# ami-iit/paper_gorbani_2025_humanoids_multi-rate-mpc-ironcub

Measured on AMD Instinct MI355X. Metric: MPC solves/sec (whole node) + p50 single-solve latency, iRonCub paper horizon, higher is better.
Workload: dtype f64

## Files before the change

paper_gorbani_2025_humanoids_multi-rate-mpc-ironcub_amd/build.py:

```python
from __future__ import annotations

import os
import shutil
import subprocess

HERE = os.path.dirname(os.path.abspath(__file__))
CSRC = os.path.join(HERE, "csrc")
LIB_PATH = os.path.join(HERE, "libvsmpc.so")
SOLVE = "vsmpc_kernels.hip"
SOURCES = [SOLVE, "vsmpc_dispatch.hip", "vsmpc_rollout.hip", "vsmpc_capi.hip", "vsmpc_capi_solve.hip", "vsmpc_capi_debug.hip",
           "vsmpc_capi_rollout.hip", "vsmpc_jet.hip", "vsmpc_provider.hip", "vsmpc_runtime.hip", "vsmpc_certify.hip"]
HEADERS = ["vsmpc_device.hpp", "vsmpc_launch.hpp", "vsmpc_host.hpp", "vsmpc_p0.hpp", "vsmpc_smem.hpp", "vsmpc_p1_syrk.hpp", "vsmpc_p1_struct.hpp",
           "vsmpc_p3.hpp", "vsmpc_p4.hpp", "vsmpc_p5.hpp", "vsmpc_panel_asm.inc",
           "vsmpc_structure.hpp", "vsmpc_rt_core.hpp", "vsmpc_rt_sens.hpp", "vsmpc_rt_adjoint.hpp", "vsmpc_solve_body.inc", "vsmpc_jet_device.hpp", "vsmpc_horizons.def", os.path.join("..", "..", "include", "vsmpc.h"),
           os.path.join("..", "..", "include", "vsmpc_jet.h")]


DEFAULT_HORIZONS = ((17, 7, 12), (34, 14, 24), (21, 9, 15))
HORIZONS_DEF = os.path.join(CSRC, "vsmpc_horizons.def")


def horizons():
    env = os.environ.get("VSMPC_HORIZONS", "").strip()
    if not env:
        return DEFAULT_HORIZONS
    out = []
    for item in env.split(";"):
        n, ns, hc = (int(v) for v in item.split(","))
        out.append((n, ns, hc))
    return tuple(out)


def write_horizons_def() -> bool:
    text = ("// Horizons (nIter, nIterSmall, controlHorizon) with a kernel instantiation: one X(...) line each.\n"
            "// Written by build.py (DEFAULT_HORIZONS or VSMPC_HORIZONS); the first two are BASELINE.json's configurations.\n"
            + "".join(f"X({n}, {ns}, {hc})\n" for n, ns, hc in horizons()))
    old = open(HORIZONS_DEF).read() if os.path.exists(HORIZONS_DEF) else None
    if old != text:
        with open(HORIZONS_DEF, "w") as f:
            f.write(text)
        return True
    return False


def _hipcc() -> str:
    for cand in (shutil.which("hipcc"), "/opt/rocm/bin/hipcc"):
        if cand and os.path.exists(cand):
            return cand
    raise RuntimeError("hipcc not found: the vsmpc HIP library cannot be built")


OBJ_DIR = os.path.join(HERE, "build")


SCHED_MAX_ILP = ["-mllvm", "-amdgpu-sched-strategy=max-ilp"]
SMALL_SCHED = SCHED_MAX_ILP


def _units():
    units = []
    for n, ns, hc in horizons():
        sched = SCHED_MAX_ILP if n <= 24 else []
        for st in (0, 1):
            units.append((f"kernels_{n}_{ns}_{hc}_{'diag' if st else 'prod'}", SOLVE,
                          [f"-DVS_TU_HORIZON={n},{ns},{hc}", f"-DVS_TU_STAMPS={st}"] + sched))
        for form in (0, 1):
            units.append((f"kernels_{n}_{ns}_{hc}_tuned_{'struct' if form else 'syrk'}", SOLVE,
                          [f"-DVS_TU_HORIZON={n},{ns},{hc}", "-DVS_TU_STAMPS=2", f"-DVS_TU_FORM={form}"] + sched))
        units.append((f"kernels_{n}_{ns}_{hc}_small", SOLVE, [f"-DVS_TU_HORIZON={n},{ns},{hc}", "-DVS_TU_STAMPS=3"] + SMALL_SCHED))
    for src in SOURCES:
        if src != SOLVE:
            units.append((os.path.splitext(src)[0], src, []))
    return units


def _deps(src):
    return [os.path.join(CSRC, src)] + [os.path.join(CSRC, h) for h in HEADERS] + [os.path.abspath(__file__)]


def _extra_flags():
    return os.environ.get("VSMPC_HIPCC_FLAGS", "").split()


def needs_build() -> bool:
    if not os.path.exists(LIB_PATH):
        return True
    t = os.path.getmtime(LIB_PATH)
    deps = [os.path.join(CSRC, s) for s in SOURCES + HEADERS] + [os.path.abspath(__file__)]
    return any(os.path.getmtime(d) > t for d in deps)


def build_library(force: bool = False, verbose: bool = False, jobs: int | None = None) -> str:
    from concurrent.futures import ThreadPoolExecutor
    changed = write_horizons_def()
    if not force and not changed and not needs_build():
        return LIB_PATH
    os.makedirs(OBJ_DIR, exist_ok=True)
    hipcc = _hipcc()
    base = [hipcc, "--offload-arch=gfx950", "-O3", "-std=c++17", "-fPIC", "-c"] + _extra_flags()
    if verbose:
        base.insert(1, "-Rpass-analysis=kernel-resource-usage")
    todo, objs = [], []
    for name, src, flags in _units():
        obj = os.path.join(OBJ_DIR, name + ".o")
        stamp = obj + ".flags"
        cmd = base + flags + [os.path.join(CSRC, src), "-o", obj]
        objs.append(obj)
        flagtext = " ".join(cmd)
        fresh = (not force and os.path.exists(obj) and os.path.exists(stamp) and open(stamp).read() == flagtext
                 and all(os.path.getmtime(d) <= os.path.getmtime(obj) for d in _deps(src)))
        if not fresh:
            todo.append((cmd, stamp, flagtext))

    def run(item):
        cmd, stamp, flagtext = item
        res = subprocess.run(cmd, capture_output=True, text=True)
        if res.returncode == 0:
            with open(stamp, "w") as f:
                f.write(flagtext)
        return cmd, res

    jobs = jobs or int(os.environ.get("VSMPC_BUILD_JOBS", "0")) or min(8, os.cpu_count() or 1)
    with ThreadPoolExecutor(max_workers=jobs) as pool:
        results = list(pool.map(run, todo))
    for cmd, res in results:
        if res.returncode != 0:
            raise RuntimeError("hipcc failed: " + " ".join(cmd) + "\n" + res.stdout + res.stderr)
        if verbose:
            print(res.stderr)
    keep = {os.path.basename(o) for o in objs}
    for f in os.listdir(OBJ_DIR):
        if f.endswith(".o") and f not in keep:
            os.remove(os.path.join(OBJ_DIR, f))
    link = [hipcc, "--offload-arch=gfx950", "-shared", "-fPIC", "-Wl,-rpath,/opt/rocm/lib", "-o", LIB_PATH] + objs
    res = subprocess.run(link, capture_output=True, text=True)
    if res.returncode != 0:
        raise RuntimeError("link failed:\n" + res.stdout + res.stderr)
    return LIB_PATH


def build_bindings(force: bool = False) -> str | None:
    try:
        import pybind11
    except ImportError:
        return None
    import sysconfig
    src = os.path.join(CSRC, "bindings_mpc.cpp")
    out = os.path.join(HERE, "bindingsMPC" + (sysconfig.get_config_var("EXT_SUFFIX") or ".so"))
    deps = [src, os.path.join(HERE, "..", "include", "VariableSamplingMPC.hpp"), os.path.join(HERE, "..", "include", "vsmpc.h")]
    if not force and os.path.exists(out) and all(os.path.getmtime(d) <= os.path.getmtime(out) for d in deps):
        return out
    build_library()
    cmd = ["g++", "-O2", "-std=c++17", "-shared", "-fPIC", f"-I{pybind11.get_include()}",
           f"-I{sysconfig.get_paths()['include']}", src, "-o", out, f"-L{HERE}", "-lvsmpc",
           "-Wl,-rpath,$ORIGIN", "-Wl,-rpath,/opt/rocm/lib"]
    res = subprocess.run(cmd, capture_output=True, text=True)
    if res.returncode != 0:
        raise RuntimeError("bindingsMPC build failed:\n" + res.stdout + res.stderr)
    return out


if __name__ == "__main__":
    print(build_library(force=True, verbose=True))
```

paper_gorbani_2025_humanoids_multi-rate-mpc-ironcub_amd/csrc/vsmpc_kernels.hip:

```cpp
#include <atomic>

#include "vsmpc_launch.hpp"
#include "vsmpc_p0.hpp"
#include "vsmpc_p1_syrk.hpp"
#include "vsmpc_p1_struct.hpp"
#include "vsmpc_p3.hpp"
#include "vsmpc_p4.hpp"
#include "vsmpc_p5.hpp"

#if !defined(VS_TU_HORIZON) || !defined(VS_TU_STAMPS)
#error "one unit per horizon and kind: -DVS_TU_HORIZON=N,NS,HC -DVS_TU_STAMPS=0|1, =2 -DVS_TU_FORM=0|1, or =3 (build.py)"
#endif
#if VS_TU_STAMPS == 2 && !defined(VS_TU_FORM)
#error "a unit of the tuned kind holds one condensing form: -DVS_TU_FORM=0|1"
#endif

namespace vsmpc {

template <class D, int K0 = 0, int K1 = NJC>
VS_DEV void p0_joint_reduction(double* __restrict__ sm, int lane) {
    using S = Smem<D>;
    static_assert(VSMPC_IN_LANG == VSMPC_IN_LLIN + 24, "Lambda_lin and Lambda_ang are adjacent in the record");
    const double* sIn = sm + S::oIn;
    const double* sCfg = sm + S::oCfg;
    double* sBj = sm + S::oBj;
    double* sQR = sm + S::oQR;
    const int c = lane < 6 ? lane : 6;
    double a[8];
    if constexpr (K0 == 0) {
#pragma unroll
        for (int j = 0; j < 8; ++j) {
            const double isw = fast_rsqrt(sCfg[CFG_WJ + j]);
            const double lam = sIn[VSMPC_IN_LLIN + (c < 6 ? c : 0) * 8 + j];
            const double bq = sCfg[CFG_WREG] * sIn[VSMPC_IN_QERR + j];
            a[j] = (c < 6 ? lam : bq) * isw;
            if (lane == 0) sQR[S::QR_ISW + j] = isw;
        }
    } else {
#pragma unroll
        for (int j = 0; j < 8; ++j) a[j] = sQR[S::QR_A + 8 * c + j];
    }
#pragma unroll
    for (int k = K0; k < K1; ++k) {
        double s0 = a[k] * a[k], s1 = 0.0;
#pragma unroll
        for (int i = k + 1; i < 8; i += 2) {
            s1 = fma(a[i], a[i], s1);
            if (i + 1 < 8) s0 = fma(a[i + 1], a[i + 1], s0);
        }
        const double s = s0 + s1;
        const double sk = readlane_f64(s, k), xk = readlane_f64(a[k], k);
        const bool nz = sk > 1e-300;
        const double rs = fast_rsqrt(nz ? sk : 1.0);
        const double nrm = nz ? sk * rs : 0.0;
        const double alpha = xk >= 0.0 ? -nrm : nrm;
        const double beta = nz ? rs * fast_rcp(nrm + fabs(xk)) : 0.0;
        double v[8];
        v[k] = xk - alpha;
#pragma unroll
        for (int i = k + 1; i < 8; ++i) v[i] = readlane_f64(a[i], k);
        double w0 = v[k] * a[k], w1 = 0.0;
#pragma unroll
        for (int i = k + 1; i < 8; i += 2) {
            w1 = fma(v[i], a[i], w1);
            if (i + 1 < 8) w0 = fma(v[i + 1], a[i + 1], w0);
        }
        const double w = (w0 + w1) * beta;
        const bool behind = lane > k;
#pragma unroll
        for (int i = k; i < 8; ++i) a[i] = behind ? fma(-w, v[i], a[i]) : a[i];
        a[k] = lane == k ? alpha : a[k];
        if (lane == 0) {
#pragma unroll
            for (int i = 0; i < 8; ++i) sQR[S::QR_V + 8 * k + i] = i >= k ? v[i] : 0.0;
            sQR[S::QR_BETA + k] = beta;
        }
    }
    if constexpr (K1 < NJC) {
        if (lane < 7) {
#pragma unroll
            for (int j = 0; j < 8; ++j) sQR[S::QR_A + 8 * lane + j] = a[j];
        }
        return;
    }
    if (lane < 6) {
        const int row = lane < 3 ? 3 + lane : 6 + lane;
#pragma unroll
        for (int k = 0; k < NJC; ++k) sBj[row * NJ + k] = k <= lane ? a[k] : 0.0;
    } else if (lane == 6) {
#pragma unroll
        for (int k = 0; k < NJC; ++k) sQR[S::QR_GY + k] = a[k];
        sQR[S::QR_NS + 0] = -a[6];
        sQR[S::QR_NS + 1] = -a[7];
    }
}

template <class D, int K1 = NJC, int K0 = 0>
VS_DEV void joint_expand(const double* __restrict__ sQR, const double* __restrict__ y, double (&u)[8]) {
    using S = Smem<D>;
    if constexpr (K1 == NJC) {
#pragma unroll
        for (int i = 0; i < NJC; ++i) u[i] = y[i];
        u[6] = sQR[S::QR_NS + 0];
        u[7] = sQR[S::QR_NS + 1];
    }
#pragma unroll
    for (int k = K1 - 1; k >= K0; --k) {
        double t = 0.0;
#pragma unroll
        for (int i = k; i < 8; ++i) t = fma(sQR[S::QR_V + 8 * k + i], u[i], t);
        t *= sQR[S::QR_BETA + k];
#pragma unroll
        for (int i = k; i < 8; ++i) u[i] = fma(-t, sQR[S::QR_V + 8 * k + i], u[i]);
    }
    if constexpr (K0 == 0) {
#pragma unroll
        for (int i = 0; i < 8; ++i) u[i] *= sQR[S::QR_ISW + i];
    }
}

struct SolveArgs {
    DevCfg cfg;
    const double* in;
    int batch;
    int pad_;
    double* xout;
    double* fmout;
    int* status_out;
    int* iters_out;
    double* dbgM;
    double* dbgL;
    unsigned long long* stamps;
};
VS_DEV const SolveArgs* late_args() {
    const SolveArgs* ka = reinterpret_cast<const SolveArgs*>(
        (const void*)__builtin_amdgcn_kernarg_segment_ptr());
    asm volatile("" : "+s"(ka));
    return ka;
}

template <class D, bool STAMPS, int FORM = 0>
__global__ __launch_bounds__(D::BLOCK, D::WG_PER_CU) void solve_kernel(DevCfg cfg, const double* __restrict__ in, int batch,
                                                         double* xout_, double* fmout_, int* status_out_,
                                                         int* iters_out_, double* dbgM_, double* dbgL_,
                                                         unsigned long long* stamps_) {
    constexpr bool TUNED = false;
    constexpr bool SMALL = false;
    const double* const tun = nullptr;
#include "vsmpc_solve_body.inc"
}

template <class D, int FORM = 0>
__global__ __launch_bounds__(D::BLOCK, D::WG_PER_CU) void solve_kernel_tuned(DevCfg cfg, const double* __restrict__ in, int batch,
                                                         double* xout_, double* fmout_, int* status_out_,
                                                         int* iters_out_, double* dbgM_, double* dbgL_,
                                                         unsigned long long* stamps_, const double* __restrict__ tun) {
    constexpr bool STAMPS = false;
    constexpr bool TUNED = true;
    constexpr bool SMALL = false;
#include "vsmpc_solve_body.inc"
}

template <class D, bool STAMPS>
__global__ __launch_bounds__(D::BLOCK, D::WG_PER_CU) void solve_kernel_small(DevCfg cfg, const double* __restrict__ in, int batch,
                                                         double* xout_, double* fmout_, int* status_out_,
                                                         int* iters_out_, double* dbgM_, double* dbgL_,
                                                         unsigned long long* stamps_) {
    constexpr bool TUNED = false;
    constexpr bool SMALL = true;
    constexpr int FORM = 1;
    const double* const tun = nullptr;
#include "vsmpc_solve_body.inc"
}

template <class D, bool STAMPS, int FORM>
static hipError_t launch_solve_f(const DevCfg& cfg, const double* d_in, int batch, double* d_x, double* d_fm,
                                 int* d_status, int* d_iters, double* dbgM, double* dbgL,
                                 unsigned long long* stamps, hipStream_t stream) {
    static std::atomic<bool> attr_set[MAX_DEVICES];
    constexpr size_t lds = FORM == 1 ? Smem<D>::bytes_struct : Smem<D>::bytes;
    const hipError_t e = allow_dynamic_lds(reinterpret_cast<const void*>(&solve_kernel<D, STAMPS, FORM>), attr_set, lds);
    if (e != hipSuccess) return e;
    hipLaunchKernelGGL((solve_kernel<D, STAMPS, FORM>), dim3(batch), dim3(D::BLOCK), lds, stream,
                       cfg, d_in, batch, d_x, d_fm, d_status, d_iters, dbgM, dbgL, stamps);
    return hipGetLastError();
}

template <int N, int NS, int HC, bool STAMPS>
hipError_t launch_solve_dims(int form, const DevCfg& cfg, const double* d_in, int batch, double* d_x, double* d_fm,
                             int* d_status, int* d_iters, double* dbgM, double* dbgL, unsigned long long* stamps,
                             hipStream_t stream) {
    using D = Dims<N, NS, HC>;
    if constexpr (D::STRUCT_P1) {
        if (form != 2) {
            return launch_solve_f<D, STAMPS, 1>(cfg, d_in, batch, d_x, d_fm, d_status, d_iters, dbgM, dbgL, stamps, stream);
        }
    }
    return launch_solve_f<D, STAMPS, 0>(cfg, d_in, batch, d_x, d_fm, d_status, d_iters, dbgM, dbgL, stamps, stream);
}

template <int N, int NS, int HC>
hipError_t launch_solve_small_dims(const DevCfg& cfg, const double* d_in, int batch, double* d_x, double* d_fm, int* d_status,
                                   int* d_iters, unsigned long long* stamps, hipStream_t stream) {
    using D = Dims<N, NS, HC>;
    if constexpr (!has_small_kind<D>()) {
        return hipErrorInvalidValue;
    } else {
        static std::atomic<bool> attr_set[2][MAX_DEVICES];
        constexpr size_t lds = Smem<D, true>::bytes_struct;
        static_assert(lds <= 160 * 1024, "the small-batch kind takes the LDS of one CU");
        auto go = [&](auto stc) {
            constexpr bool ST = decltype(stc)::value;
            const hipError_t e = allow_dynamic_lds(reinterpret_cast<const void*>(&solve_kernel_small<D, ST>), attr_set[ST], lds);
            if (e != hipSuccess) return e;
            hipLaunchKernelGGL((solve_kernel_small<D, ST>), dim3(batch), dim3(D::BLOCK), lds, stream, cfg, d_in, batch, d_x, d_fm,
                               d_status, d_iters, static_cast<double*>(nullptr), static_cast<double*>(nullptr), stamps);
            return hipGetLastError();
        };
        return stamps != nullptr ? go(std::true_type{}) : go(std::false_type{});
    }
}

template <int N, int NS, int HC, int FORM>
hipError_t launch_solve_tuned_dims(const DevCfg& cfg, const double* d_in, const double* d_tun, int batch, double* d_x,
                                   double* d_fm, int* d_status, int* d_iters, hipStream_t stream) {
    using D = Dims<N, NS, HC>;
    if constexpr (FORM == 1 && !D::STRUCT_P1) {
        return hipErrorInvalidValue;
    } else {
        static std::atomic<bool> attr_set[MAX_DEVICES];
        constexpr size_t lds = FORM == 1 ? Smem<D>::bytes_struct : Smem<D>::bytes;
        static_assert(D::WG_PER_CU < 2 || lds <= 80 * 1024, "the tuned kind keeps two workgroups per CU");
        const hipError_t e = allow_dynamic_lds(reinterpret_cast<const void*>(&solve_kernel_tuned<D, FORM>), attr_set, lds);
        if (e != hipSuccess) return e;
        hipLaunchKernelGGL((solve_kernel_tuned<D, FORM>), dim3(batch), dim3(D::BLOCK), lds, stream, cfg, d_in, batch, d_x, d_fm,
                           d_status, d_iters, static_cast<double*>(nullptr), static_cast<double*>(nullptr),
                           static_cast<unsigned long long*>(nullptr), d_tun);
        return hipGetLastError();
    }
}

#define VS_INSTANTIATE_SOLVE(N, NS, HC, ST)                                                                              \
    template hipError_t launch_solve_dims<N, NS, HC, ST>(int, const DevCfg&, const double*, int, double*, double*, int*, \
                                                         int*, double*, double*, unsigned long long*, hipStream_t);
#define VS_INSTANTIATE_TUNED(N, NS, HC, F)                                                                                 \
    template hipError_t launch_solve_tuned_dims<N, NS, HC, F>(const DevCfg&, const double*, const double*, int, double*, \
                                                              double*, int*, int*, hipStream_t);
#define VS_TU_APPLY(M, ...) M(__VA_ARGS__)
#define VS_INSTANTIATE_SMALL(N, NS, HC)                                                                              \
    template hipError_t launch_solve_small_dims<N, NS, HC>(const DevCfg&, const double*, int, double*, double*, int*, int*, \
                                                           unsigned long long*, hipStream_t);
#if VS_TU_STAMPS == 3
VS_TU_APPLY(VS_INSTANTIATE_SMALL, VS_TU_HORIZON)
#elif VS_TU_STAMPS == 2
VS_TU_APPLY(VS_INSTANTIATE_TUNED, VS_TU_HORIZON, VS_TU_FORM)
#elif VS_TU_STAMPS
VS_TU_APPLY(VS_INSTANTIATE_SOLVE, VS_TU_HORIZON, true)
#else
VS_TU_APPLY(VS_INSTANTIATE_SOLVE, VS_TU_HORIZON, false)
#endif

}
```

paper_gorbani_2025_humanoids_multi-rate-mpc-ironcub_amd/csrc/vsmpc_solve_body.inc:

```
#define VS_STAMP(i)                                                                         \
    do {                                                                                    \
        if constexpr (STAMPS) {                                                             \
            unsigned long long* st_ = late_args()->stamps;                                  \
            if (tid == 0 && st_ != nullptr) st_[size_t(blockIdx.x) * 16 + (i)] = __builtin_amdgcn_s_memtime(); \
        }                                                                                   \
    } while (0)
    unsigned long long t_acc[6] = {0, 0, 0, 0, 0, 0};
    unsigned long long t_mark = 0, stamp_t1 = 0, rt0 = 0;
    if constexpr (STAMPS) rt0 = __builtin_amdgcn_s_memrealtime();
#define VS_TIC()                                                     \
    do {                                                             \
        if constexpr (STAMPS) t_mark = __builtin_amdgcn_s_memtime(); \
    } while (0)
#define VS_TOC(i)                                                          \
    do {                                                                   \
        if constexpr (STAMPS) {                                            \
            const unsigned long long t_now = __builtin_amdgcn_s_memtime(); \
            t_acc[i] += t_now - t_mark;                                    \
            t_mark = t_now;                                                \
        }                                                                  \
    } while (0)
    using S = Smem<D, SMALL>;
    static_assert(!SMALL || (FORM == 1 && !TUNED), "the small-batch kind is the structured form of the shared kind");
    constexpr bool FUSED_DISPATCH = FORM == 1;
// ... 368 lines not shown
                    }
                }
            }
            if (nnodes == 1)
                for (int i = ptid; i < 2 * D::YS; i += D::BLOCK) sYm[18 * D::YS + i] = 0.0;
        };
        auto syrk_fixed = [&](auto nks_c, auto nact_c) __attribute__((always_inline)) {
            constexpr int NKS = decltype(nks_c)::value, NACT = decltype(nact_c)::value;
            if constexpr (NACT > 0) {
                double ha[SYRK_DIST], hb[SYRK_DIST];
#pragma unroll
                for (int ks = 0; ks < SYRK_DIST; ++ks) {
                    ha[ks] = slot_a(NACT - 1)[ks * 4 * D::YS];
                    hb[ks] = slot_b(NACT - 1)[ks * 4 * D::YS];
                }
#pragma unroll
                for (int q = NACT - 1; q >= 0; --q) {
                    const int qn = q > 0 ? q - 1 : 0;
                    syrk_slot<D, NKS, true>(acc[q], slot_a(q), slot_b(q), ha, hb, slot_a(qn), slot_b(qn));
                }
            }
        };
        if constexpr (UNROLLED) {
            static_for<0, NPASS>([&](auto mc) __attribute__((always_inline)) {
                constexpr int m = decltype(mc)::value;
                constexpr int nnodes = (2 * m + 1 < D::N) ? 2 : 1;
                VS_TIC();
                rec_pass(m, nnodes, sY);
                VS_TOC(0);
                __syncthreads();
                VS_TOC(1);
                syrk_fixed(std::integral_constant<int, nnodes == 2 ? 9 : 5>{}, std::integral_constant<int, nact_max<D>(m)>{});
                VS_TOC(2);
                __syncthreads();
            });
        } else {
            static_for<0, PassGroups<D>::count()>([&](auto gc) __attribute__((always_inline)) {
                constexpr PassGroups<D> pg{};
                constexpr int g = decltype(gc)::value;
#pragma unroll 1
                for (int m = pg.start[g]; m < pg.end[g]; ++m) {
                    VS_TIC();
                    rec_pass(m, pg.nks[g] == 9 ? 2 : 1, sY);
                    VS_TOC(0);
                    __syncthreads();
                    VS_TOC(1);
                    syrk_fixed(std::integral_constant<int, pg.nks[g]>{}, std::integral_constant<int, pg.nact[g]>{});
                    VS_TOC(2);
                    __syncthreads();
                }
            });
        }
        VS_TIC();
    }
    if constexpr (!FUSED_DISPATCH) VS_STAMP(2);
    VS_REFRESH_IDS();
    if constexpr (D::WG_PER_CU == 1) pin_tiles_agpr<TPW>(acc);

    constexpr int PVT = D::PVT;
    const int crow = (lane >> 4) * 17 + (lane & 15);
    const int lrow = (lane & 15) * 17 + (lane >> 4);
    double* dbgM = STAMPS ? late_args()->dbgM : nullptr;
    double* dbgL = STAMPS ? late_args()->dbgL : nullptr;
    double* dbgLi = dbgL != nullptr ? dbgL + size_t(inst) * D::NP * D::NP : nullptr;
    if (STAMPS && !FUSED_DISPATCH && dbgM != nullptr) {
#pragma unroll
        for (int q = 0; q < TPW; ++q) {
            if (kTileTab<D, PIPE>.forms(q * D::NWAVES + wave, wave)) {
                const int ti_q = kTileTab<D, PIPE>.ti[q * D::NWAVES + wave], tj_q = kTileTab<D, PIPE>.tj[q * D::NWAVES + wave];
                d4 tmp = acc[q];
                if (ti_q == tj_q || ti_q >= PVT) {
#pragma unroll
                    for (int r = 0; r < 4; ++r)
                        tmp[r] += input_cost_term<D>(sCfg, smem + S::oQR + S::QR_GY, sVprev, 16 * ti_q + (lane >> 4) + 4 * r,
                                                     16 * tj_q + (lane & 15));
                }
#pragma unroll
                for (int r = 0; r < 4; ++r) {
                    const int gr = 16 * ti_q + (lane >> 4) + 4 * r, gc = 16 * tj_q + (lane & 15);
                    if (gc <= gr) dbgM[size_t(inst) * D::NP * D::NP + size_t(gr) * D::NP + gc] = tmp[r];
                }
            }
        }
    }
    if constexpr (!FUSED_DISPATCH) VS_STAMP(3);
    VS_REFRESH_IDS();
    if constexpr (!FUSED_DISPATCH)
    switch (wave) {
        case 0: cholesky_wave<D, TPW, 0, STAMPS, PIPE>(sCfg, acc, Lb, sInvD, smem + S::oQR + S::QR_GY, sVprev, sFlags, sXinv, sW, dbgLi, lane, crow, lrow, sZ); break;
        case 1: cholesky_wave<D, TPW, 1, STAMPS, PIPE>(sCfg, acc, Lb, sInvD, smem + S::oQR + S::QR_GY, sVprev, sFlags, sXinv, sW, dbgLi, lane, crow, lrow, sZ); break;
        case 2: cholesky_wave<D, TPW, 2, STAMPS, PIPE>(sCfg, acc, Lb, sInvD, smem + S::oQR + S::QR_GY, sVprev, sFlags, sXinv, sW, dbgLi, lane, crow, lrow, sZ); break;
        default: cholesky_wave<D, TPW, 3, STAMPS, PIPE>(sCfg, acc, Lb, sInvD, smem + S::oQR + S::QR_GY, sVprev, sFlags, sXinv, sW, dbgLi, lane, crow, lrow, sZ); break;
    }
    static_assert(D::NWAVES == 4, "wave-specialised phases are instantiated for four wavefronts");
    if (STAMPS && dbgLi != nullptr) {
        if constexpr (!FUSED_DISPATCH) {
#pragma unroll
            for (int q = 0; q < TPW; ++q) {
                const int ti_q = kTileTab<D, PIPE>.ti[q * D::NWAVES + wave], tj_q = kTileTab<D, PIPE>.tj[q * D::NWAVES + wave];
                if (kTileTab<D, PIPE>.holds(q * D::NWAVES + wave, wave) && tj_q < PVT && ti_q > tj_q) {
#pragma unroll
                    for (int r = 0; r < 4; ++r)
                        dbgLi[size_t(16 * ti_q + (lane >> 4) + 4 * r) * D::NP + 16 * tj_q + (lane & 15)] = acc[q][r];
                }
            }
        }
        for (int e = tid; e < (D::NP - 16 * PVT) * (D::NP - 16 * PVT); e += D::BLOCK) {
            const int gr = 16 * PVT + e / (D::NP - 16 * PVT), gc = 16 * PVT + e % (D::NP - 16 * PVT);
            if (gc <= gr) dbgLi[size_t(gr) * D::NP + gc] = Lb[lower_at<D>(gr, gc)];
        }
    }

    VS_STAMP(4);
    VS_REFRESH_IDS();
    if constexpr (D::WG_PER_CU == 1) pin_tiles_agpr<TPW>(acc);
    const bool hold = sIn[VSMPC_IN_HOLD] != 0.0;
    constexpr int PV = D::PVT;
    auto init_corner_rhs = [&]() {
        if (tid >= 16 * PV && tid < D::NP) sW[tid] = tid < D::NZ ? -Lb[lower_at<D>(D::NZ, tid)] : 0.0;
    };
    init_corner_rhs();
    if (tid < D::NP) sZ[tid] = (hold && tid >= D::NZ - 4 && tid < D::NZ) ? sVprev[tid - (D::NZ - 4)] : 0.0;
    __syncthreads();

    auto sweep_tile = [&](int p, bool prescribed) {
        if (wave == 0) {
            const int j = lane & 15;
            const int gj = 16 * p + j;
            const double* Tpp = Lb + tile_off<D>(p, p) + j;
            double colv[16];
#pragma unroll
            for (int k = 0; k < 16; ++k) {
                const double t = Tpp[k * 17];
                colv[k] = k >= j ? t : 0.0;
            }
            double w = sW[gj];
            const bool fix = (gj >= D::NZ) || (gj >= D::NU && (prescribed || (hold && gj >= D::NZ - 4)));
            const double inv_eff = fix ? 0.0 : sInvD[gj];
            const double zadd = (fix && gj < D::NZ) ? sZ[gj] : 0.0;
            double z = 0.0;
#pragma unroll
            for (int k = 15; k >= 0; --k) {
                const double zk = readlane_f64(fma(w, inv_eff, zadd), k);
                z = (j == k) ? zk : z;
                w = fma(-colv[k], zk, w);
            }
            if (lane < 16) sZ[gj] = z;
        }
        __syncthreads();
        if (p > PV) {
            if (tid >= 16 * PV && tid < 16 * p) {
                const double* T = Lb + tile_off<D>(p, tid >> 4) + (tid & 15);
                const double* zp = sZ + 16 * p;
                double a2 = 0.0;
#pragma unroll
                for (int k = 0; k < 16; ++k) a2 += T[k * 17] * zp[k];
                sW[tid] -= a2;
            }
            __syncthreads();
        }
    };

    constexpr bool DUALQP = S::DUALQP;
    if constexpr (DUALQP) {
        constexpr int PL = D::NT - 1, KL = D::NZ - 16 * PL;
        static_assert(KL == D::NV - 16 && KL >= 4, "pins live in the last tile row");
        const double* X6 = sXinv + PV * D::TS;
        const double* L76 = Lb + tile_off<D>(PL, PV);
        const double* L77 = Lb + tile_off<D>(PL, PL);
        if (wave == 0) {
            const int j = lane & 15;
            const int gj = 16 * PL + j;
            const double* Tpp = L77 + j;
            double colv[KL], l76[KL], x6[16];
#pragma unroll
            for (int k = 0; k < KL; ++k) {
                const double t = Tpp[k * 17];
                colv[k] = k >= j ? t : 0.0;
                l76[k] = L76[k * 17 + j];
            }
#pragma unroll
            for (int i = 0; i < 16; ++i) x6[i] = X6[i * 17 + j];
            double w = sW[gj];
            double w6 = sW[16 * PV + j];
            const bool fix = (j >= KL) || (hold && j >= KL - 4);
            const double inv_eff = fix ? 0.0 : sInvD[gj];
            const double zadd = (fix && j < KL) ? sZ[gj] : 0.0;
            double z = 0.0;
#pragma unroll
            for (int k = KL - 1; k >= 0; --k) {
                const double zk = readlane_f64(fma(w, inv_eff, zadd), k);
                z = (j == k) ? zk : z;
                w = fma(-colv[k], zk, w);
                w6 = fma(-l76[k], zk, w6);
            }
            double z6 = 0.0;
#pragma unroll
            for (int i = 0; i < 16; ++i) z6 = fma(x6[i], readlane_f64(w6, i), z6);
            if (lane < 16) { sZ[gj] = z; sZ[16 * PV + j] = z6; }
        } else {
            dual_setup_beside_sweep<D>(wave, lane);
        }
    } else if constexpr (S::DUAL3) {
        static_assert(D::NT - 1 == PV + 2, "three throttle tile rows");
        double x2[16];
        const double* L22d = Lb + tile_off_c<D>(PV + 2, PV + 2);
        const double* inv2 = sInvD + D::NU + 32;
        if (wave == 1) tile_inverse_rows<0, 8>(L22d, inv2, x2, lane);
        sweep_tile(PV + 2, false);
        auto sweep_tile_x = [&](int p, const double* Xp) {
            if (wave == 0) {
                const int j = lane & 15;
                double z0 = 0.0, z1 = 0.0;
#pragma unroll
                for (int k = 0; k < 16; k += 2) {
                    z0 = fma(Xp[k * 17 + j], sW[16 * p + k], z0);
                    z1 = fma(Xp[(k + 1) * 17 + j], sW[16 * p + k + 1], z1);
                }
                if (lane < 16) sZ[16 * p + j] = z0 + z1;
            }
            __syncthreads();
            if (p > PV) {
                if (tid >= 16 * PV && tid < 16 * p) {
                    const double* T = Lb + tile_off<D>(p, tid >> 4) + (tid & 15);
                    const double* zp = sZ + 16 * p;
                    double a2 = 0.0;
#pragma unroll
                    for (int k = 0; k < 16; ++k) a2 += T[k * 17] * zp[k];
                    sW[tid] -= a2;
                }
                __syncthreads();
            }
        };
        if (wave == 1) tile_inverse_rows<8, 13>(L22d, inv2, x2, lane);
        sweep_tile_x(PV + 1, smem + S::oDual3T0);
        if (wave == 1) {
            tile_inverse_rows<13, 16>(L22d, inv2, x2, lane);
            if (lane < 16) {
#pragma unroll
                for (int i = 0; i < 16; ++i) smem[S::oDual3T1 + i * 17 + lane] = x2[i];
            }
        }
        sweep_tile_x(PV, sXinv + PV * D::TS);
    } else {
#pragma unroll 1
        for (int p = D::NT - 1; p >= PV; --p) sweep_tile(p, false);
    }
    if (wave == 0) {
        const bool valid = lane < D::NV;
        const double v = sZ[D::NU + (valid ? lane : 0)];
        const bool fixed = hold && lane >= D::NV - 4;
        const double tolv = 1e-12 * (1.0 + fabs(v));
        const bool viol = valid && !fixed && (v < sCfg[CFG_VMIN] - tolv || v > sCfg[CFG_VMAX] + tolv);
        const unsigned long long vm = __ballot(viol);
        if (lane == 0) { sFlags[3] = __popcll(vm); sFlags[1] = VSMPC_STATUS_SOLVED; sFlags[2] = 1; }
        if constexpr (DUALQP) {
            if (lane == 0) sFlags[4] = int(unsigned(vm));
        }
    }
    __syncthreads();
    const bool need_qp = sFlags[3] != 0;
    VS_STAMP(5);
    VS_REFRESH_IDS();

#ifdef VS_DIAG_QP
    for (int i = 0; i < 4; ++i) t_acc[i] = 0;
#endif
    if (need_qp) {
#ifdef VS_DIAG_QP
        box_qp<D>(sFlags[3], hold, wave, STAMPS ? t_acc : nullptr);
#else
        box_qp<D>(sFlags[3], hold, wave);
#endif
        __syncthreads();
        VS_STAMP(6);
        VS_REFRESH_IDS();
        if constexpr (D::NU % 16 != 0) {
            init_corner_rhs();
            __syncthreads();
#pragma unroll 1
            for (int p = D::NT - 1; p >= PV; --p) sweep_tile(p, true);
        }
    } else {
        VS_STAMP(6);
    }
    switch (wave) {
        case 0:
            if constexpr (PIPE) p5_wave0_jets<D>(smem, lane);
            else backsub_wave<D, TPW, 0, PIPE>(acc, sW, sZ, sXinv, sU, lane);
            break;
        case 1: backsub_wave<D, TPW, 1, PIPE>(acc, sW, sZ, sXinv, sU, lane); break;
        case 2: backsub_wave<D, TPW, 2, PIPE>(acc, sW, sZ, sXinv, sU, lane); break;
        default: backsub_wave<D, TPW, 3, PIPE>(acc, sW, sZ, sXinv, sU, lane); break;
    }
    if (tid < D::NV) sV[tid] = sZ[D::NU + tid];
    __syncthreads();

    VS_STAMP(7);
    VS_REFRESH_IDS();
#ifdef VS_DIAG_P6
    for (int i = 0; i < 4; ++i) t_acc[i] = 0;
    VS_TIC();
#define VS_P6_TOC(i) VS_TOC(i)
#else
#define VS_P6_TOC(i) do { } while (0)
#endif
    const SolveArgs* ka = late_args();
    double* xout = ka->xout;
    double* fmout = ka->fmout;
    int* status_out = ka->status_out;
    int* iters_out = ka->iters_out;
    double u8[8] = {0.0, 0.0, 0.0, 0.0, 0.0, 0.0, 0.0, 0.0};
    constexpr int JX_SPLIT = PIPE ? 3 : NJC;
    if (PIPE && wave == 3 && lane < D::HC) joint_expand<D, NJC, JX_SPLIT>(smem + S::oQR, sZ + NJC * lane, u8);
    {
        constexpr int ROWS = PIPE ? 6 : NX;
        constexpr int NE = ROWS * D::N, RND = (NE + D::BLOCK - 1) / D::BLOCK;
#pragma unroll
        for (int rd = 0; rd < RND; ++rd) {
            const int e0 = tid + rd * D::BLOCK, ec = e0 < NE ? e0 : NE - 1;
            const int k = ec / ROWS, rr = ec - k * ROWS;
            const int r = PIPE ? (rr < 3 ? 3 + rr : 6 + rr) : rr;
            const int e = NX * k + r;
            const int jb = joint_block_of_stage<D>(k);
            const int tb = throttle_block_of_stage<D>(k);
            const int vq = tb == 0 ? D::NV - 4 : 4 * (tb - 1);
            double f = sC[r];
#pragma unroll
            for (int c = 0; c < NJC; ++c) f += sBj[r * NJ + c] * sZ[NJC * jb + c];
#pragma unroll
            for (int c = 0; c < NTH; ++c) f += sBt[r * NTH + c] * sV[vq + c];
            if (e0 < NE) sF[e] = f;
        }
    }
    __syncthreads();
    VS_P6_TOC(0);
    {
        constexpr int CHK = D::N > 20 ? 9 : 6, NCH = (D::N + CHK - 1) / CHK;
        double jT = 0.0, jTd = 0.0, jon = 0.0, ja = 0.0, jb = 0.0;
        double Sk[9], hh[3] = {0.0, 0.0, 0.0};
        double cm0 = 0.0, cm1 = 0.0, cm2 = 0.0, cce = 0.0, cx = 0.0, cee = 0.0;
        const int hr0m = (lane & 1) ? 9 : 3;
        const int cg = lane / 3, cr = lane - 3 * cg;
        const int cxr = (cg ? 6 : 0) + cr, chr0 = cg ? 9 : 3, cer = (cg ? 23 : 20) + cr;
        constexpr bool JETS_EARLY = PIPE;
        constexpr int JOFF = JETS_EARLY ? 0 : 1;
        if (!JETS_EARLY && wave == 0 && lane < NTH) {
            jon = sA[(12 + lane) * NX + 16 + lane]; ja = sA[(16 + lane) * NX + 12 + lane]; jb = sA[(16 + lane) * NX + 16 + lane];
            jT = sIn[VSMPC_IN_X0 + 12 + lane]; jTd = sIn[VSMPC_IN_X0 + 16 + lane];
            sX[12 + lane] = jT;
            sX[16 + lane] = jTd;
        }
        if (wave == 1 && lane < 2) {
#pragma unroll
            for (int r = 0; r < 3; ++r) {
                hh[r] = sIn[VSMPC_IN_X0 + hr0m + r];
                sX[hr0m + r] = hh[r];
#pragma unroll
                for (int c = 0; c < 3; ++c) Sk[3 * r + c] = sA[(hr0m + r) * NX + hr0m + c];
            }
        }
        if (wave == 2 && lane < 6) {
            cm0 = sA[cxr * NX + chr0]; cm1 = sA[cxr * NX + chr0 + 1]; cm2 = sA[cxr * NX + chr0 + 2];
            cce = sC[cer];
            cx = sIn[VSMPC_IN_X0 + cxr]; cee = sIn[VSMPC_IN_X0 + cer];
            sX[cxr] = cx;
            sX[cer] = cee;
        }
        static_assert(D::NUO <= D::NWAVES * D::NP, "joint increments fit the partial-sum array");
        if (wave == 3 && lane < D::HC) {
            if constexpr (PIPE) joint_expand<D, JX_SPLIT, 0>(smem + S::oQR, sZ + NJC * lane, u8);
            else joint_expand<D>(smem + S::oQR, sZ + NJC * lane, u8);
#pragma unroll
            for (int i = 0; i < 8; ++i) sU[NJ * lane + i] = u8[i];
        }
        if (wave == 3 && xout != nullptr) {
            double2* xo = reinterpret_cast<double2*>(xout + size_t(inst) * D::NVAR);
            for (int i = lane; i < D::NUO / 2; i += 64) xo[D::NXS / 2 + i] = make_double2(sU[2 * i], sU[2 * i + 1]);
            if (lane < D::NV / 2) {
                const int e = 2 * lane, b = e >> 2, c = e & 3;
                const int q = b == 0 ? D::NV - 4 + c : 4 * (b - 1) + c;
                xo[(D::NXS + D::NUO) / 2 + lane] = make_double2(sV[q], sV[q + 1]);
            }
        }

        static_for<0, NCH + 1 + JOFF>([&](auto scst) __attribute__((always_inline)) {
            constexpr int st = decltype(scst)::value;
            if constexpr (!JETS_EARLY && st < NCH) {
                if (wave == 0 && lane < NTH) {
                    constexpr int k0 = st * CHK;
                    double fa[CHK], fb[CHK], dtk[CHK];
#pragma unroll
                    for (int u = 0; u < CHK; ++u) {
                        const int k = (k0 + u < D::N) ? k0 + u : D::N - 1;
                        fa[u] = sF[NX * k + 12 + lane];
                        fb[u] = sF[NX * k + 16 + lane];
                        dtk[u] = sDt[k];
                    }
#pragma unroll
                    for (int u = 0; u < CHK; ++u) {
                        const double dT = fma(jon, jTd, fa[u]);
                        const double dTd = fma(ja, jT, fma(jb, jTd, fb[u]));
                        jT = fma(dtk[u], dT, jT);
                        jTd = fma(dtk[u], dTd, jTd);
                        if (k0 + u < D::N) {
                            sX[NX * (k0 + u + 1) + 12 + lane] = jT;
                            sX[NX * (k0 + u + 1) + 16 + lane] = jTd;
                        }
                    }
                }
            }
            if constexpr (PIPE && st == 1) {
                if (wave == 3 && fmout != nullptr && lane < VSMPC_FM_SIZE) {
                    double v;
                    if (lane < 8) v = sU[lane];
                    else if (lane < 12) v = sV[D::NV - 4 + (lane - 8)];
                    else if (lane < 16) v = Jet::throttle_of_v(sV[D::NV - 4 + (lane - 12)]);
                    else if (lane < 20) v = sX[NX + 12 + (lane - 16)];
                    else v = sX[NX + 16 + (lane - 20)];
                    fmout[size_t(inst) * VSMPC_FM_SIZE + lane] = v;
                }
            }
            if constexpr (st >= JOFF && st - JOFF < NCH) {
                if (wave == 1) {
                    constexpr int k0 = (st - JOFF) * CHK;
                    constexpr int kn = k0 + CHK < D::N ? CHK : D::N - k0;
                    if (lane < 6 * kn) {
                        const int k = k0 + lane / 6, rr = lane % 6, row = rr < 3 ? 3 + rr : 6 + rr;
                        double gk = sF[NX * k + row];
#pragma unroll
                        for (int c = 0; c < NTH; ++c) gk = fma(sA[row * NX + 12 + c], sX[NX * k + 12 + c], gk);
                        sF[NX * k + row] = gk;
                    }
                    if (lane < 2) {
                        double gk[CHK][3], dtk[CHK];
#pragma unroll
                        for (int u = 0; u < CHK; ++u) {
                            const int k = (k0 + u < D::N) ? k0 + u : D::N - 1;
#pragma unroll
                            for (int r = 0; r < 3; ++r) gk[u][r] = sF[NX * k + hr0m + r];
                            dtk[u] = sDt[k];
                        }
#pragma unroll
                        for (int u = 0; u < CHK; ++u) {
                            double dh[3];
#pragma unroll
                            for (int r = 0; r < 3; ++r)
                                dh[r] = fma(Sk[3 * r], hh[0], fma(Sk[3 * r + 1], hh[1], fma(Sk[3 * r + 2], hh[2], gk[u][r])));
#pragma unroll
                            for (int r = 0; r < 3; ++r) hh[r] = fma(dtk[u], dh[r], hh[r]);
                            if (k0 + u < D::N) {
#pragma unroll
                                for (int r = 0; r < 3; ++r) sX[NX * (k0 + u + 1) + hr0m + r] = hh[r];
                            }
                        }
                    }
                }
            }
            if constexpr (st >= JOFF + 1 && st - JOFF - 1 < NCH) {
                if (wave == 2 && lane < 6) {
                    constexpr int k0 = (st - JOFF - 1) * CHK;
                    double hk[CHK][3], dtk[CHK];
#pragma unroll
                    for (int u = 0; u < CHK; ++u) {
                        const int k = (k0 + u < D::N) ? k0 + u : D::N - 1;
#pragma unroll
                        for (int c = 0; c < 3; ++c) hk[u][c] = sX[NX * k + chr0 + c];
                        dtk[u] = sDt[k];
                    }
#pragma unroll
                    for (int u = 0; u < CHK; ++u) {
                        const double dx = fma(cm0, hk[u][0], fma(cm1, hk[u][1], cm2 * hk[u][2]));
                        cee = fma(dtk[u], cx + cce, cee);
                        cx = fma(dtk[u], dx, cx);
                        if (k0 + u < D::N) {
                            sX[NX * (k0 + u + 1) + cxr] = cx;
                            sX[NX * (k0 + u + 1) + cer] = cee;
                        }
                    }
                }
            }
            if constexpr (st + 1 < NCH + 1 + JOFF) __syncthreads();
            if constexpr (st == 0) VS_P6_TOC(1);
        });
    }
    __syncthreads();
    VS_P6_TOC(2);
    VS_STAMP(8);
    VS_REFRESH_IDS();

    if (xout != nullptr) {
        double2* xo = reinterpret_cast<double2*>(xout + size_t(inst) * D::NVAR);
        for (int i = tid; i < D::NXS / 2; i += D::BLOCK) xo[i] = make_double2(sX[2 * i], sX[2 * i + 1]);
    }
    if (!PIPE && fmout != nullptr && tid < VSMPC_FM_SIZE) {
        double v;
        if (tid < 8) v = sU[tid];
        else if (tid < 12) v = sV[D::NV - 4 + (tid - 8)];
        else if (tid < 16) v = Jet::throttle_of_v(sV[D::NV - 4 + (tid - 12)]);
        else if (tid < 20) v = sX[NX + 12 + (tid - 16)];
        else v = sX[NX + 16 + (tid - 20)];
        fmout[size_t(inst) * VSMPC_FM_SIZE + tid] = v;
    }
    if (tid == 0) {
        int st = sFlags[1];
        if (sFlags[0]) st = VSMPC_STATUS_NUMERICAL;
        status_out[inst] = st;
        if (iters_out != nullptr) iters_out[inst] = sFlags[2];
    }
    VS_P6_TOC(3);
    VS_STAMP(9);
    if constexpr (STAMPS) {
        unsigned long long* st_ = late_args()->stamps;
        if (tid == 0 && st_ != nullptr) {
#if defined(VS_DIAG_P3) && !defined(VS_DIAG_P6)
            for (int i = 0; i < 4; ++i) t_acc[i] = vs_diag_p3[i];
#endif
            t_acc[5] = __builtin_amdgcn_s_memrealtime() - rt0;
            t_acc[4] = rt0;
            for (int i = 0; i < 6; ++i) st_[size_t(blockIdx.x) * 16 + 10 + i] = t_acc[i];
        }
    }
#undef VS_STAMP
#undef VS_REFRESH_IDS
#undef VS_TIC
#undef VS_TOC
```

Baseline: 8.157 million.

## Restructure final rollout phase into single-wave streamed chains without per-chunk barriers

Replaces the multi-wave chunked pipeline of the state rollout (jets on wave 0, angular momentum on wave 1, CoM on wave 2, separated by a __syncthreads per chunk) with a design where wave 0 first integrates the jet states, then one barrier, then a fused chain (momentum plus CoM in six lanes) streams through the horizon with double-buffered register preloads. The jet coupling term is folded into the parallel forcing computation ahead of time. This removes many block-wide barriers and the wave-to-wave handoff latency, at the cost of serialising the jet and chain recurrences on a single wave and doing more redundant per-lane arithmetic.

```diff
diff --git a/paper_gorbani_2025_humanoids_multi-rate-mpc-ironcub_amd/build.py b/paper_gorbani_2025_humanoids_multi-rate-mpc-ironcub_amd/build.py
--- a/paper_gorbani_2025_humanoids_multi-rate-mpc-ironcub_amd/build.py
+++ b/paper_gorbani_2025_humanoids_multi-rate-mpc-ironcub_amd/build.py
@@ -11,7 +11,7 @@
 SOURCES = [SOLVE, "vsmpc_dispatch.hip", "vsmpc_rollout.hip", "vsmpc_capi.hip", "vsmpc_capi_solve.hip", "vsmpc_capi_debug.hip",
            "vsmpc_capi_rollout.hip", "vsmpc_jet.hip", "vsmpc_provider.hip", "vsmpc_runtime.hip", "vsmpc_certify.hip"]
 HEADERS = ["vsmpc_device.hpp", "vsmpc_launch.hpp", "vsmpc_host.hpp", "vsmpc_p0.hpp", "vsmpc_smem.hpp", "vsmpc_p1_syrk.hpp", "vsmpc_p1_struct.hpp",
-           "vsmpc_p3.hpp", "vsmpc_p4.hpp", "vsmpc_p5.hpp", "vsmpc_panel_asm.inc",
+           "vsmpc_p3.hpp", "vsmpc_p4.hpp", "vsmpc_p5.hpp", "vsmpc_p6.hpp", "vsmpc_panel_asm.inc",
            "vsmpc_structure.hpp", "vsmpc_rt_core.hpp", "vsmpc_rt_sens.hpp", "vsmpc_rt_adjoint.hpp", "vsmpc_solve_body.inc", "vsmpc_jet_device.hpp", "vsmpc_horizons.def", os.path.join("..", "..", "include", "vsmpc.h"),
            os.path.join("..", "..", "include", "vsmpc_jet.h")]
 
diff --git a/paper_gorbani_2025_humanoids_multi-rate-mpc-ironcub_amd/csrc/vsmpc_kernels.hip b/paper_gorbani_2025_humanoids_multi-rate-mpc-ironcub_amd/csrc/vsmpc_kernels.hip
--- a/paper_gorbani_2025_humanoids_multi-rate-mpc-ironcub_amd/csrc/vsmpc_kernels.hip
+++ b/paper_gorbani_2025_humanoids_multi-rate-mpc-ironcub_amd/csrc/vsmpc_kernels.hip
@@ -7,6 +7,7 @@
 #include "vsmpc_p3.hpp"
 #include "vsmpc_p4.hpp"
 #include "vsmpc_p5.hpp"
+#include "vsmpc_p6.hpp"
 
 #if !defined(VS_TU_HORIZON) || !defined(VS_TU_STAMPS)
 #error "one unit per horizon and kind: -DVS_TU_HORIZON=N,NS,HC -DVS_TU_STAMPS=0|1, =2 -DVS_TU_FORM=0|1, or =3 (build.py)"
diff --git a/paper_gorbani_2025_humanoids_multi-rate-mpc-ironcub_amd/csrc/vsmpc_p6.hpp b/paper_gorbani_2025_humanoids_multi-rate-mpc-ironcub_amd/csrc/vsmpc_p6.hpp
--- /dev/null
+++ b/paper_gorbani_2025_humanoids_multi-rate-mpc-ironcub_amd/csrc/vsmpc_p6.hpp
@@ -0,0 +1,122 @@
+#pragma once
+#include "vsmpc_p5.hpp"
+
+namespace vsmpc {
+
+template <class D>
+struct P6Groups {
+    static constexpr int GRP = D::N <= 18 ? D::N : 9;
+    static constexpr int NG = (D::N + GRP - 1) / GRP;
+};
+
+template <class D>
+VS_DEV void p6_jets_stream(const double* __restrict__ sIn, const double* __restrict__ sA, const double* __restrict__ sF,
+                           const double* __restrict__ sDt, double* __restrict__ sX, int lane) {
+    constexpr int GRP = P6Groups<D>::GRP, NG = P6Groups<D>::NG;
+    if (lane < NTH) {
+        const double jon = sA[(12 + lane) * NX + 16 + lane], ja = sA[(16 + lane) * NX + 12 + lane], jb = sA[(16 + lane) * NX + 16 + lane];
+        double jT = sIn[VSMPC_IN_X0 + 12 + lane], jTd = sIn[VSMPC_IN_X0 + 16 + lane];
+        sX[12 + lane] = jT;
+        sX[16 + lane] = jTd;
+        double fa[2][GRP], fb[2][GRP], dtk[2][GRP];
+        auto load = [&](auto gcst) __attribute__((always_inline)) {
+            constexpr int g = decltype(gcst)::value, b = g & 1;
+#pragma unroll
+            for (int u = 0; u < GRP; ++u) {
+                const int k = (g * GRP + u < D::N) ? g * GRP + u : D::N - 1;
+                fa[b][u] = sF[NX * k + 12 + lane];
+                fb[b][u] = sF[NX * k + 16 + lane];
+                dtk[b][u] = sDt[k];
+            }
+        };
+        load(std::integral_constant<int, 0>{});
+        static_for<0, NG>([&](auto gcst) __attribute__((always_inline)) {
+            constexpr int g = decltype(gcst)::value, b = g & 1;
+            if constexpr (g + 1 < NG) load(std::integral_constant<int, g + 1>{});
+#pragma unroll
+            for (int u = 0; u < GRP; ++u) {
+                if (g * GRP + u < D::N) {
+                    const double dT = fma(jon, jTd, fa[b][u]);
+                    const double dTd = fma(ja, jT, fma(jb, jTd, fb[b][u]));
+                    jT = fma(dtk[b][u], dT, jT);
+                    jTd = fma(dtk[b][u], dTd, jTd);
+                    sX[NX * (g * GRP + u + 1) + 12 + lane] = jT;
+                    sX[NX * (g * GRP + u + 1) + 16 + lane] = jTd;
+                }
+            }
+        });
+    }
+}
+
+struct P6Chain {
+    double Sk[9], hh[3];
+    double cm0, cm1, cm2, cce, cx, cee;
+    int hr0, xr, er, r;
+};
+
+template <class D>
+VS_DEV void p6_chain_init(P6Chain& ch, const double* __restrict__ sIn, const double* __restrict__ sA,
+                          const double* __restrict__ sC, double* __restrict__ sX, int lane) {
+    const int g = lane / 3;
+    ch.r = lane - 3 * g;
+    ch.hr0 = g ? 9 : 3;
+    ch.xr = (g ? 6 : 0) + ch.r;
+    ch.er = (g ? 23 : 20) + ch.r;
+#pragma unroll
+    for (int r = 0; r < 3; ++r) {
+        ch.hh[r] = sIn[VSMPC_IN_X0 + ch.hr0 + r];
+#pragma unroll
+        for (int c = 0; c < 3; ++c) ch.Sk[3 * r + c] = sA[(ch.hr0 + r) * NX + ch.hr0 + c];
+    }
+    ch.cm0 = sA[ch.xr * NX + ch.hr0]; ch.cm1 = sA[ch.xr * NX + ch.hr0 + 1]; ch.cm2 = sA[ch.xr * NX + ch.hr0 + 2];
+    ch.cce = sC[ch.er];
+    ch.cx = sIn[VSMPC_IN_X0 + ch.xr]; ch.cee = sIn[VSMPC_IN_X0 + ch.er];
+    sX[ch.hr0 + ch.r] = sIn[VSMPC_IN_X0 + ch.hr0 + ch.r];
+    sX[ch.xr] = ch.cx;
+    sX[ch.er] = ch.cee;
+}
+
+template <class D, class Mid>
+VS_DEV void p6_chain_stream(P6Chain& ch, const double* __restrict__ sF, const double* __restrict__ sDt,
+                            double* __restrict__ sX, Mid&& after_preload) {
+    constexpr int GRP = P6Groups<D>::GRP, NG = P6Groups<D>::NG;
+    double gk[2][GRP][3], dtk[2][GRP];
+    auto load = [&](auto gcst) __attribute__((always_inline)) {
+        constexpr int g = decltype(gcst)::value, b = g & 1;
+#pragma unroll
+        for (int u = 0; u < GRP; ++u) {
+            const int k = (g * GRP + u < D::N) ? g * GRP + u : D::N - 1;
+#pragma unroll
+            for (int r = 0; r < 3; ++r) gk[b][u][r] = sF[NX * k + ch.hr0 + r];
+            dtk[b][u] = sDt[k];
+        }
+    };
+    load(std::integral_constant<int, 0>{});
+    after_preload();
+    const bool r0 = ch.r == 0, r1 = ch.r == 1;
+    static_for<0, NG>([&](auto gcst) __attribute__((always_inline)) {
+        constexpr int g = decltype(gcst)::value, b = g & 1;
+        if constexpr (g + 1 < NG) load(std::integral_constant<int, g + 1>{});
+#pragma unroll
+        for (int u = 0; u < GRP; ++u) {
+            if (g * GRP + u < D::N) {
+                const double dt = dtk[b][u];
+                const double dx = fma(ch.cm0, ch.hh[0], fma(ch.cm1, ch.hh[1], ch.cm2 * ch.hh[2]));
+                ch.cee = fma(dt, ch.cx + ch.cce, ch.cee);
+                ch.cx = fma(dt, dx, ch.cx);
+                double dh[3];
+#pragma unroll
+                for (int r = 0; r < 3; ++r)
+                    dh[r] = fma(ch.Sk[3 * r], ch.hh[0], fma(ch.Sk[3 * r + 1], ch.hh[1], fma(ch.Sk[3 * r + 2], ch.hh[2], gk[b][u][r])));
+#pragma unroll
+                for (int r = 0; r < 3; ++r) ch.hh[r] = fma(dt, dh[r], ch.hh[r]);
+                double* xn = sX + NX * (g * GRP + u + 1);
+                xn[ch.hr0 + ch.r] = r0 ? ch.hh[0] : (r1 ? ch.hh[1] : ch.hh[2]);
+                xn[ch.xr] = ch.cx;
+                xn[ch.er] = ch.cee;
+            }
+        }
+    });
+}
+
+}
diff --git a/paper_gorbani_2025_humanoids_multi-rate-mpc-ironcub_amd/csrc/vsmpc_solve_body.inc b/paper_gorbani_2025_humanoids_multi-rate-mpc-ironcub_amd/csrc/vsmpc_solve_body.inc
--- a/paper_gorbani_2025_humanoids_multi-rate-mpc-ironcub_amd/csrc/vsmpc_solve_body.inc
+++ b/paper_gorbani_2025_humanoids_multi-rate-mpc-ironcub_amd/csrc/vsmpc_solve_body.inc
@@ -694,8 +694,15 @@
     for (int i = 0; i < 4; ++i) t_acc[i] = 0;
     VS_TIC();
 #define VS_P6_TOC(i) VS_TOC(i)
+#define VS_P6_PRELOAD_DONE()                      \
+    do {                                          \
+        __builtin_amdgcn_sched_barrier(0);        \
+        __builtin_amdgcn_s_waitcnt(0xc07f);       \
+        __builtin_amdgcn_sched_barrier(0);        \
+    } while (0)
 #else
 #define VS_P6_TOC(i) do { } while (0)
+#define VS_P6_PRELOAD_DONE() do { } while (0)
 #endif
     const SolveArgs* ka = late_args();
     double* xout = ka->xout;
@@ -705,59 +712,57 @@
     double u8[8] = {0.0, 0.0, 0.0, 0.0, 0.0, 0.0, 0.0, 0.0};
     constexpr int JX_SPLIT = PIPE ? 3 : NJC;
     if (PIPE && wave == 3 && lane < D::HC) joint_expand<D, NJC, JX_SPLIT>(smem + S::oQR, sZ + NJC * lane, u8);
+    auto input_term = [&](int r, int k) __attribute__((always_inline)) {
+        const int jb = joint_block_of_stage<D>(k);
+        const int tb = throttle_block_of_stage<D>(k);
+        const int vq = tb == 0 ? D::NV - 4 : 4 * (tb - 1);
+        double f = sC[r];
+#pragma unroll
+        for (int c = 0; c < NJC; ++c) f += sBj[r * NJ + c] * sZ[NJC * jb + c];
+#pragma unroll
+        for (int c = 0; c < NTH; ++c) f += sBt[r * NTH + c] * sV[vq + c];
+        return f;
+    };
+    if constexpr (!PIPE) {
+        if (wave == 0) {
+            constexpr int NEJ = 8 * D::N, RNDJ = (NEJ + 63) / 64;
+#pragma unroll
+            for (int rd = 0; rd < RNDJ; ++rd) {
+                const int e0 = lane + rd * 64, ec = e0 < NEJ ? e0 : NEJ - 1;
+                const int k = ec >> 3, r = 12 + (ec & 7);
+                const double f = input_term(r, k);
+                if (e0 < NEJ) sF[NX * k + r] = f;
+            }
+            p6_jets_stream<D>(sIn, sA, sF, sDt, sX, lane);
+        }
+        __syncthreads();
+    }
+    P6Chain ch;
+    if constexpr (PIPE) {
+        if (wave == 0 && lane < 6) p6_chain_init<D>(ch, sIn, sA, sC, sX, lane);
+    }
     {
-        constexpr int ROWS = PIPE ? 6 : NX;
-        constexpr int NE = ROWS * D::N, RND = (NE + D::BLOCK - 1) / D::BLOCK;
+        constexpr int NE = 6 * D::N, RND = (NE + D::BLOCK - 1) / D::BLOCK;
 #pragma unroll
         for (int rd = 0; rd < RND; ++rd) {
             const int e0 = tid + rd * D::BLOCK, ec = e0 < NE ? e0 : NE - 1;
-            const int k = ec / ROWS, rr = ec - k * ROWS;
-            const int r = PIPE ? (rr < 3 ? 3 + rr : 6 + rr) : rr;
-            const int e = NX * k + r;
-            const int jb = joint_block_of_stage<D>(k);
-            const int tb = throttle_block_of_stage<D>(k);
-            const int vq = tb == 0 ? D::NV - 4 : 4 * (tb - 1);
-            double f = sC[r];
-#pragma unroll
-            for (int c = 0; c < NJC; ++c) f += sBj[r * NJ + c] * sZ[NJC * jb + c];
-#pragma unroll
-            for (int c = 0; c < NTH; ++c) f += sBt[r * NTH + c] * sV[vq + c];
-            if (e0 < NE) sF[e] = f;
+            const int k = ec / 6, rr = ec - k * 6;
+            const int r = rr < 3 ? 3 + rr : 6 + rr;
+            double gk = input_term(r, k);
+#pragma unroll
+            for (int c = 0; c < NTH; ++c) gk = fma(sA[r * NX + 12 + c], sX[NX * k + 12 + c], gk);
+            if (e0 < NE) sF[NX * k + r] = gk;
         }
     }
     __syncthreads();
     VS_P6_TOC(0);
     {
-        constexpr int CHK = D::N > 20 ? 9 : 6, NCH = (D::N + CHK - 1) / CHK;
-        double jT = 0.0, jTd = 0.0, jon = 0.0, ja = 0.0, jb = 0.0;
-        double Sk[9], hh[3] = {0.0, 0.0, 0.0};
-        double cm0 = 0.0, cm1 = 0.0, cm2 = 0.0, cce = 0.0, cx = 0.0, cee = 0.0;
-        const int hr0m = (lane & 1) ? 9 : 3;
-        const int cg = lane / 3, cr = lane - 3 * cg;
-        const int cxr = (cg ? 6 : 0) + cr, chr0 = cg ? 9 : 3, cer = (cg ? 23 : 20) + cr;
-        constexpr bool JETS_EARLY = PIPE;
-        constexpr int JOFF = JETS_EARLY ? 0 : 1;
-        if (!JETS_EARLY && wave == 0 && lane < NTH) {
-            jon = sA[(12 + lane) * NX + 16 + lane]; ja = sA[(16 + lane) * NX + 12 + lane]; jb = sA[(16 + lane) * NX + 16 + lane];
-            jT = sIn[VSMPC_IN_X0 + 12 + lane]; jTd = sIn[VSMPC_IN_X0 + 16 + lane];
-            sX[12 + lane] = jT;
-            sX[16 + lane] = jTd;
-        }
-        if (wave == 1 && lane < 2) {
-#pragma unroll
-            for (int r = 0; r < 3; ++r) {
-                hh[r] = sIn[VSMPC_IN_X0 + hr0m + r];
-                sX[hr0m + r] = hh[r];
-#pragma unroll
-                for (int c = 0; c < 3; ++c) Sk[3 * r + c] = sA[(hr0m + r) * NX + hr0m + c];
-            }
-        }
-        if (wave == 2 && lane < 6) {
-            cm0 = sA[cxr * NX + chr0]; cm1 = sA[cxr * NX + chr0 + 1]; cm2 = sA[cxr * NX + chr0 + 2];
-            cce = sC[cer];
-            cx = sIn[VSMPC_IN_X0 + cxr]; cee = sIn[VSMPC_IN_X0 + cer];
-            sX[cxr] = cx;
-            sX[cer] = cee;
+        if (wave == 0 && lane < 6) {
+            if constexpr (!PIPE) p6_chain_init<D>(ch, sIn, sA, sC, sX, lane);
+            p6_chain_stream<D>(ch, sF, sDt, sX, [&]() __attribute__((always_inline)) {
+                VS_P6_PRELOAD_DONE();
+                VS_P6_TOC(1);
+            });
         }
         static_assert(D::NUO <= D::NWAVES * D::NP, "joint increments fit the partial-sum array");
         if (wave == 3 && lane < D::HC) {
@@ -775,106 +780,17 @@
                 xo[(D::NXS + D::NUO) / 2 + lane] = make_double2(sV[q], sV[q + 1]);
             }
         }
-
-        static_for<0, NCH + 1 + JOFF>([&](auto scst) __attribute__((always_inline)) {
-            constexpr int st = decltype(scst)::value;
-            if constexpr (!JETS_EARLY && st < NCH) {
-                if (wave == 0 && lane < NTH) {
-                    constexpr int k0 = st * CHK;
-                    double fa[CHK], fb[CHK], dtk[CHK];
-#pragma unroll
-                    for (int u = 0; u < CHK; ++u) {
-                        const int k = (k0 + u < D::N) ? k0 + u : D::N - 1;
-                        fa[u] = sF[NX * k + 12 + lane];
-                        fb[u] = sF[NX * k + 16 + lane];
-                        dtk[u] = sDt[k];
-                    }
-#pragma unroll
-                    for (int u = 0; u < CHK; ++u) {
-                        const double dT = fma(jon, jTd, fa[u]);
-                        const double dTd = fma(ja, jT, fma(jb, jTd, fb[u]));
-                        jT = fma(dtk[u], dT, jT);
-                        jTd = fma(dtk[u], dTd, jTd);
-                        if (k0 + u < D::N) {
-                            sX[NX * (k0 + u + 1) + 12 + lane] = jT;
-                            sX[NX * (k0 + u + 1) + 16 + lane] = jTd;
-                        }
-                    }
-                }
-            }
-            if constexpr (PIPE && st == 1) {
-                if (wave == 3 && fmout != nullptr && lane < VSMPC_FM_SIZE) {
-                    double v;
-                    if (lane < 8) v = sU[lane];
-                    else if (lane < 12) v = sV[D::NV - 4 + (lane - 8)];
-                    else if (lane < 16) v = Jet::throttle_of_v(sV[D::NV - 4 + (lane - 12)]);
-                    else if (lane < 20) v = sX[NX + 12 + (lane - 16)];
-                    else v = sX[NX + 16 + (lane - 20)];
-                    fmout[size_t(inst) * VSMPC_FM_SIZE + lane] = v;
-                }
-            }
-            if constexpr (st >= JOFF && st - JOFF < NCH) {
-                if (wave == 1) {
-                    constexpr int k0 = (st - JOFF) * CHK;
-                    constexpr int kn = k0 + CHK < D::N ? CHK : D::N - k0;
-                    if (lane < 6 * kn) {
-                        const int k = k0 + lane / 6, rr = lane % 6, row = rr < 3 ? 3 + rr : 6 + rr;
-                        double gk = sF[NX * k + row];
-#pragma unroll
-                        for (int c = 0; c < NTH; ++c) gk = fma(sA[row * NX + 12 + c], sX[NX * k + 12 + c], gk);
-                        sF[NX * k + row] = gk;
-                    }
-                    if (lane < 2) {
-                        double gk[CHK][3], dtk[CHK];
-#pragma unroll
-                        for (int u = 0; u < CHK; ++u) {
-                            const int k = (k0 + u < D::N) ? k0 + u : D::N - 1;
-#pragma unroll
-                            for (int r = 0; r < 3; ++r) gk[u][r] = sF[NX * k + hr0m + r];
-                            dtk[u] = sDt[k];
-                        }
-#pragma unroll
-                        for (int u = 0; u < CHK; ++u) {
-                            double dh[3];
-#pragma unroll
-                            for (int r = 0; r < 3; ++r)
-                                dh[r] = fma(Sk[3 * r], hh[0], fma(Sk[3 * r + 1], hh[1], fma(Sk[3 * r + 2], hh[2], gk[u][r])));
-#pragma unroll
-                            for (int r = 0; r < 3; ++r) hh[r] = fma(dtk[u], dh[r], hh[r]);
-                            if (k0 + u < D::N) {
-#pragma unroll
-                                for (int r = 0; r < 3; ++r) sX[NX * (k0 + u + 1) + hr0m + r] = hh[r];
-                            }
-                        }
-                    }
-                }
-            }
-            if constexpr (st >= JOFF + 1 && st - JOFF - 1 < NCH) {
-                if (wave == 2 && lane < 6) {
-                    constexpr int k0 = (st - JOFF - 1) * CHK;
-                    double hk[CHK][3], dtk[CHK];
-#pragma unroll
-                    for (int u = 0; u < CHK; ++u) {
-                        const int k = (k0 + u < D::N) ? k0 + u : D::N - 1;
-#pragma unroll
-                        for (int c = 0; c < 3; ++c) hk[u][c] = sX[NX * k + chr0 + c];
-                        dtk[u] = sDt[k];
-                    }
-#pragma unroll
-                    for (int u = 0; u < CHK; ++u) {
-                        const double dx = fma(cm0, hk[u][0], fma(cm1, hk[u][1], cm2 * hk[u][2]));
-                        cee = fma(dtk[u], cx + cce, cee);
-                        cx = fma(dtk[u], dx, cx);
-                        if (k0 + u < D::N) {
-                            sX[NX * (k0 + u + 1) + cxr] = cx;
-                            sX[NX * (k0 + u + 1) + cer] = cee;
-                        }
-                    }
-                }
-            }
-            if constexpr (st + 1 < NCH + 1 + JOFF) __syncthreads();
-            if constexpr (st == 0) VS_P6_TOC(1);
-        });
+        if constexpr (PIPE) {
+            if (wave == 3 && fmout != nullptr && lane < VSMPC_FM_SIZE) {
+                double v;
+                if (lane < 8) v = sU[lane];
+                else if (lane < 12) v = sV[D::NV - 4 + (lane - 8)];
+                else if (lane < 16) v = Jet::throttle_of_v(sV[D::NV - 4 + (lane - 12)]);
+                else if (lane < 20) v = sX[NX + 12 + (lane - 16)];
+                else v = sX[NX + 16 + (lane - 20)];
+                fmout[size_t(inst) * VSMPC_FM_SIZE + lane] = v;
+            }
+        }
     }
     __syncthreads();
     VS_P6_TOC(2);
@@ -917,3 +833,5 @@
 #undef VS_REFRESH_IDS
 #undef VS_TIC
 #undef VS_TOC
+#undef VS_P6_TOC
+#undef VS_P6_PRELOAD_DONE
```

Result: no change. 8.236 million, median of 6 (+1.0%).
